# marbl/meryl

Hardware: AMD Instinct MI355X
Metric: distinct k-mers counted/sec (whole node) (higher is better)
Workload: dtype u64; 1 GPU; meryl count k=21 on synthetic short reads: 66666667 x 150 bp reads per GPU (10.00 Gbp per GPU, 30x of a 333333334 bp genome, 0.5% substitutions, 0.01% N), inputs resident in HBM; k=21, reads_per_gpu=66666667, bases_per_gpu=10066666717, n_distinct=1181289506, parallelism=1 GPU, transport=none (one GPU), n_instances=8648488363, w_prefix=18

## Files before the change

meryl_amd/build.py:

```python
import os
import shutil
import subprocess
import sys

HERE = os.path.dirname(os.path.abspath(__file__))
CSRC = os.path.join(HERE, "csrc")
LIB = os.path.join(HERE, "libmeryl_gpu_count.so")
SOURCES = ["mgc_kmer.hip", "mgc_sort.hip", "mgc_scan.hip", "mgc_finish.hip", "mgc_misc.hip", "mgc_parse.hip",
           "mgc_encode.hip", "mgc_decode.hip", "mgc_merge.hip", "mgc_merge_many.hip", "mgc_lookup.hip", "mgc_filter.hip", "mgc_import.hip", "mgc_analyze.hip", "mgc_value_hist.hip", "mgc_positions.hip",
           "mgc_api.cpp", "mgc_textfile.cpp", "mgc_import.cpp", "mgc_analyze.cpp", "mgc_dbfile.cpp", "mgc_positions.cpp", "mgc_count.cpp", "mgc_stream.cpp", "mgc_eval.cpp", "mgc_runs.cpp", "mgc_node.cpp", "meryl_db.cpp", "meryl_seq.cpp"]
HEADERS = ["mgc_device.h", "mgc_common.hpp", "mgc_compact.hpp", "mgc_bases.hpp", "mdb_layout.h", "mdb_statistics.hpp", "mgc_session.hpp", "mgc_devbuf.hpp", "mgc_dbfile.hpp", "mgc_hist_list.hpp", "mgc_clock.hpp", "mgc_chunk_ring.hpp", "mgc_bgzf.hpp", "mgc_runs.hpp", "mgc_lookup_dev.hpp", "mgc_import_dev.hpp", "mgc_analyze_dev.hpp", "mgc_positions_dev.hpp", "mgc_fastx.hpp", "mgc_label.hpp", "mgc_selector.hpp", "mgc_value.hpp", "mgc_route.hpp", "mgc_group_route.hpp",
           os.path.join("..", "..", "include", "meryl_gpu_count.h"),
           os.path.join("..", "..", "include", "meryl_db.h"), os.path.join("..", "..", "include", "meryl_seq.h"),
           os.path.join("..", "..", "include", "meryl_lookup.h"), os.path.join("..", "..", "include", "meryl_import.h"),
           os.path.join("..", "..", "include", "meryl_analyze.h"), os.path.join("..", "..", "include", "meryl_positions.h")]
OBJDIR = os.path.join(HERE, "build")
CFLAGS = ["--offload-arch=gfx950", "-O3", "-std=c++17", "-fPIC", "-pthread", "-Wall", "-Wno-unused-function"]
LFLAGS = ["--offload-arch=gfx950", "-shared", "-fPIC", "-pthread", "-no-hip-rt"]


def hipcc():
    for cand in (os.environ.get("HIPCC"), shutil.which("hipcc"), "/opt/rocm/bin/hipcc"):
        if cand and os.path.exists(cand):
            return cand
    raise RuntimeError("hipcc not found: the native library cannot be built")


def _sources():
    return [f for f in SOURCES if os.path.exists(os.path.join(CSRC, f))]


def _header_mtime():
    deps = [os.path.join(CSRC, f) for f in HEADERS if os.path.exists(os.path.join(CSRC, f))]
    deps.append(os.path.abspath(__file__))
    return max(os.path.getmtime(d) for d in deps)


def _obj(f):
    return os.path.join(OBJDIR, f + ".o")


def _stale_objects(force=False):
    ht = _header_mtime()
    out = []
    for f in _sources():
        o = _obj(f)
        if force or not os.path.exists(o) or os.path.getmtime(o) < max(os.path.getmtime(os.path.join(CSRC, f)), ht):
            out.append(f)
    return out


def _stale():
    if not os.path.exists(LIB):
        return True
    t = os.path.getmtime(LIB)
    if max([_header_mtime()] + [os.path.getmtime(os.path.join(CSRC, f)) for f in _sources()]) <= t:
        return False
    if _stale_objects():
        return True
    return any(os.path.getmtime(_obj(f)) > t for f in _sources())


CLI = os.path.join(HERE, "bin", "meryl")
LOOKUP_CLI = os.path.join(HERE, "bin", "meryl-lookup")
IMPORT_CLI = os.path.join(HERE, "bin", "meryl-import")
ANALYZE_CLI = os.path.join(HERE, "bin", "meryl-analyze")
POSITION_LOOKUP_CLI = os.path.join(HERE, "bin", "position-lookup")


def _build_front_end(source, out, force, verbose, headers=()):
    src = os.path.join(CSRC, source)
    newest = max(os.path.getmtime(os.path.join(CSRC, f)) for f in (source,) + tuple(headers))
    if (not force and os.path.exists(out) and os.path.getmtime(out) >= newest
            and os.path.getmtime(out) >= os.path.getmtime(LIB)):
        return out
    os.makedirs(os.path.dirname(out), exist_ok=True)
    rocm_lib = os.path.join(os.environ.get("ROCM_PATH", "/opt/rocm"), "lib")
    tmp = "%s.tmp%d" % (out, os.getpid())
    cmd = [hipcc(), "-O2", "-std=c++17", "-pthread", src, "-o", tmp, "-L" + HERE, "-lmeryl_gpu_count",
           "-Wl,-rpath,$ORIGIN/..", "-L" + rocm_lib, "-lamdhip64", "-Wl,-rpath," + rocm_lib, "-lz"]
    if verbose:
        print(" ".join(cmd), file=sys.stderr)
    subprocess.check_call(cmd)
    os.replace(tmp, out)
    return out


def build_cli(force=False, verbose=False):
    return _build_front_end("meryl_main.cpp", CLI, force, verbose)


def build_lookup_cli(force=False, verbose=False):
    return _build_front_end("meryl_lookup_main.cpp", LOOKUP_CLI, force, verbose, ("mgc_fastx.hpp",))


def build_import_cli(force=False, verbose=False):
    return _build_front_end("meryl_import_main.cpp", IMPORT_CLI, force, verbose)


def build_analyze_cli(force=False, verbose=False):
    return _build_front_end("meryl_analyze_main.cpp", ANALYZE_CLI, force, verbose)


def build_position_lookup_cli(force=False, verbose=False):
    return _build_front_end("position_lookup_main.cpp", POSITION_LOOKUP_CLI, force, verbose, ("mgc_fastx.hpp",))


def build(force=False, verbose=False):
    if not force and not _stale():
        build_cli(False, verbose)
        build_lookup_cli(False, verbose)
        build_import_cli(False, verbose)
        build_analyze_cli(False, verbose)
        build_position_lookup_cli(False, verbose)
        return LIB
    os.makedirs(OBJDIR, exist_ok=True)
    todo = _stale_objects(force)
    procs = []
    for f in todo:
        tmp = "%s.tmp%d" % (_obj(f), os.getpid())
        cmd = [hipcc()] + CFLAGS + ["-c", os.path.join(CSRC, f), "-o", tmp]
        if verbose:
            print(" ".join(cmd), file=sys.stderr)
        procs.append((f, tmp, cmd, subprocess.Popen(cmd)))
    failed = []
    for f, tmp, cmd, p in procs:
        if p.wait() != 0:
            failed.append(f)
        else:
            os.replace(tmp, _obj(f))
    if failed:
        raise subprocess.CalledProcessError(1, "hipcc -c " + " ".join(failed))
    tmp = "%s.tmp%d" % (LIB, os.getpid())
    cmd = [hipcc()] + LFLAGS + ["-o", tmp] + [_obj(f) for f in _sources()] + ["-lz"]
    if verbose:
        print(" ".join(cmd), file=sys.stderr)
    subprocess.check_call(cmd)
    os.replace(tmp, LIB)
    build_cli(True, verbose)
    build_lookup_cli(True, verbose)
    build_import_cli(True, verbose)
    build_analyze_cli(True, verbose)
    build_position_lookup_cli(True, verbose)
    return LIB


if __name__ == "__main__":
    print(build(force="--force" in sys.argv, verbose=True))
```

meryl_amd/csrc/mgc_finish.hip:

```cpp
#include "mgc_common.hpp"

#include <algorithm>
#include <type_traits>
#include <vector>

namespace mgc {


constexpr int RL_BLOCK = 256;
constexpr u64 RL_INF   = ~0ull;
template <typename K> struct RlTile { static constexpr int KPT = 16; };
template <> struct RlTile<K128>     { static constexpr int KPT = 8;  };

struct RleWs {
  u64 *total, *tile_offs, *tile_next, *scratch;
  u64  num_tiles;
};
static inline RleWs rle_ws(void *d_ws, uint64_t n, uint32_t key_words) {
  const uint64_t tile = (uint64_t)RL_BLOCK * (key_words == 2 ? RlTile<K128>::KPT : RlTile<u64>::KPT);
  RleWs w;
  w.num_tiles = (n + tile - 1) / tile;
  w.total     = reinterpret_cast<u64 *>(d_ws);
  w.tile_offs = w.total + 8;
  w.tile_next = w.tile_offs + w.num_tiles + 1;
  w.scratch   = w.tile_next + w.num_tiles + 1;
  return w;
}
size_t rle_workspace_bytes(uint64_t n) {
  const uint64_t t = (n + 2047) / 2048;
  return (size_t)(8 + 2 * (t + 1) + scan_scratch_elems(t + 1)) * sizeof(uint64_t);
}

template <typename K>
__global__ __launch_bounds__(RL_BLOCK)
void rle_count_kernel(const K *__restrict__ in, u64 n, u64 *__restrict__ tile_cnt, u64 *__restrict__ tile_first) {
  constexpr int KPT = RlTile<K>::KPT, TILE = RL_BLOCK * KPT;
  __shared__ u32 s_cnt[RL_BLOCK / 64];
  __shared__ u64 s_min[RL_BLOCK / 64];
  const u64 tile_base = (u64)blockIdx.x * TILE;
  u32 c = 0;
  u64 first = RL_INF;
#pragma unroll
  for (int j = 0; j < KPT; j++) {
    const u64 idx = tile_base + (u64)j * RL_BLOCK + threadIdx.x;
    if (idx < n) {
      const K key = in[idx];
      const bool head = (idx == 0) || KeyOps<K>::ne(in[idx - 1], key);
      if (head) { c++; if (idx < first) first = idx; }
    }
  }
#pragma unroll
  for (int d = 32; d >= 1; d >>= 1) {
    c += __shfl_down(c, d);
    const u64 o = __shfl_down(first, d);
    first = (o < first) ? o : first;
  }
  if (lane_id() == 0) { s_cnt[wave_id()] = c; s_min[wave_id()] = first; }
  __syncthreads();
  if (threadIdx.x == 0) {
    u32 tc = 0; u64 tf = RL_INF;
    for (int i = 0; i < RL_BLOCK / 64; i++) { tc += s_cnt[i]; tf = (s_min[i] < tf) ? s_min[i] : tf; }
    tile_cnt[blockIdx.x]   = tc;
    tile_first[blockIdx.x] = tf;
  }
}

__global__ void rle_set_tail_kernel(u64 *__restrict__ tile_offs, u64 *__restrict__ tile_next, u64 num_tiles, u64 n,
                                    const u64 *__restrict__ total) {
  tile_offs[num_tiles] = *total;
  tile_next[num_tiles] = n;
}

__device__ __forceinline__ u32 rl_pad(u32 i) { return i + (i >> 4); }

template <typename K>
__global__ __launch_bounds__(RL_BLOCK)
void rle_emit_kernel(const K *__restrict__ in, u64 n, const u64 *__restrict__ tile_offs,
                     const u64 *__restrict__ tile_next, const u64 *__restrict__ d_out_base, K *__restrict__ out_keys,
                     u32 *__restrict__ out_counts) {
  const u64 out_base0 = d_out_base ? *d_out_base : 0ull;
  constexpr int RL_KPT = RlTile<K>::KPT, RL_TILE = RL_BLOCK * RL_KPT;
  __shared__ K s_keys[RL_TILE + 1 + (RL_TILE + 1) / 16 + 1];
  __shared__ u32 s_tmp[RL_BLOCK / 64 + 1];
  __shared__ u64 s_wmin[RL_BLOCK / 64];
  const u32 tid = threadIdx.x, lane = lane_id(), w = wave_id();
  const u64 tile_base = (u64)blockIdx.x * RL_TILE;

  if (tid == 0) s_keys[rl_pad(0)] = (tile_base > 0) ? in[tile_base - 1] : KeyOps<K>::zero();
#pragma unroll
  for (int j = 0; j < RL_KPT; j++) {
    const u32 i   = (u32)j * RL_BLOCK + tid;
    const u64 idx = tile_base + i;
    s_keys[rl_pad(i + 1)] = (idx < n) ? in[idx] : KeyOps<K>::zero();
  }
  __syncthreads();

  K keys[RL_KPT];
  u32 flags = 0;
  K prev = s_keys[rl_pad(tid * RL_KPT)];
#pragma unroll
  for (int j = 0; j < RL_KPT; j++) {
    const u32 i   = tid * RL_KPT + j;
    const u64 idx = tile_base + i;
    keys[j] = s_keys[rl_pad(i + 1)];
    const bool head = (idx < n) && ((idx == 0) || KeyOps<K>::ne(keys[j], prev));
    flags |= (head ? 1u : 0u) << j;
    prev = keys[j];
  }

  const u32 c = __popc(flags);
  u32 tile_heads;
  const u32 slot0 = block_excl_scan<RL_BLOCK, u32>(c, s_tmp, &tile_heads);

  const u64 fh = flags ? (tile_base + (u64)tid * RL_KPT + (u32)(__ffs(flags) - 1)) : RL_INF;
  u64 x = fh;
#pragma unroll
  for (int d = 1; d < 64; d <<= 1) {
    const u64 y = __shfl_down(x, d);
    if ((int)lane + d < 64) x = (y < x) ? y : x;
  }
  if (lane == 0) s_wmin[w] = x;
  __syncthreads();
  u64 after = tile_next[blockIdx.x + 1];
  for (int ww = RL_BLOCK / 64 - 1; ww > (int)w; ww--) after = (s_wmin[ww] < after) ? s_wmin[ww] : after;
  u64 e = __shfl_down(x, 1);
  if (lane == 63) e = RL_INF;
  u64 next = (e < after) ? e : after;

  const u64 out_base = out_base0 + tile_offs[blockIdx.x] + slot0;
#pragma unroll
  for (int j = RL_KPT - 1; j >= 0; j--) {
    if ((flags >> j) & 1u) {
      const u64 idx  = tile_base + (u64)tid * RL_KPT + j;
      const u64 slot = out_base + __popc(flags & ((1u << j) - 1u));
      out_keys[slot]   = keys[j];
      out_counts[slot] = (u32)(next - idx);
      next = idx;
    }
  }
}

hipError_t launch_rle_count(const void *d_sorted, uint64_t n, uint32_t key_words, void *d_ws, hipStream_t st) {
  RleWs w = rle_ws(d_ws, n, key_words);
  if (n == 0) return hipMemsetAsync(w.total, 0, sizeof(u64), st);
  if (key_words == 2)
    hipLaunchKernelGGL(rle_count_kernel<K128>, dim3((uint32_t)w.num_tiles), dim3(RL_BLOCK), 0, st,
                       reinterpret_cast<const K128 *>(d_sorted), (u64)n, w.tile_offs, w.tile_next);
  else
    hipLaunchKernelGGL(rle_count_kernel<u64>, dim3((uint32_t)w.num_tiles), dim3(RL_BLOCK), 0, st,
                       reinterpret_cast<const u64 *>(d_sorted), (u64)n, w.tile_offs, w.tile_next);
  MGC_CHECK(hipGetLastError());
  MGC_CHECK(scan_u64_exclusive(w.tile_offs, w.num_tiles, w.scratch, w.total, st));
  MGC_CHECK(scan_u64_min_reverse(w.tile_next, w.num_tiles, w.scratch, (u64)n, st));
// ... 508 lines not shown
          won |= w ? (1u << j) : 0u;
          pending |= (act && !w && !dup) ? (1u << j) : 0u;
        }
      }
      while (pending) {
#pragma unroll
        for (int j = 0; j < KPT; j++) {
          if ((pending >> j) & 1u) {
            hh[j] = (hh[j] + 1) & smask;
            const u32 old = atomicCAS(&tk[hh[j]], EMPTY, (comp[j] << CNTB) | 1u);
            const bool w = old == EMPTY, dup = (old >> CNTB) == comp[j];
            if (dup) atomicAdd(&tk[hh[j]], 1u);
            if (w) won |= 1u << j;
            if (w || dup) pending &= ~(1u << j);
          }
        }
      }
      {
        u64 wm[KPT];
        u32 tot = 0;
#pragma unroll
        for (int j = 0; j < KPT; j++) { wm[j] = __ballot((won >> j) & 1u); tot += (u32)__popcll(wm[j]); }
        u32 base = 0;
        if (lane == 0) base = atomicAdd(&s_nd, tot);
        base = (u32)__builtin_amdgcn_readfirstlane((int)base);
#pragma unroll
        for (int j = 0; j < KPT; j++) {
          if (wm[j]) {
            if ((won >> j) & 1u)
              lst[base + __builtin_amdgcn_mbcnt_hi((u32)(wm[j] >> 32), __builtin_amdgcn_mbcnt_lo((u32)wm[j], 0u))] = (unsigned short)hh[j];
            base += (u32)__popcll(wm[j]);
          }
        }
      }
      }
      __syncthreads();
      HC_STAMP(1);
    }

    const u32 b1 = (R >= 2) ? bc[1] : 0u, b2 = (R >= 3) ? bc[2] : 0u, b3 = (R >= 4) ? bc[3] : 0u;
    const u64 a = a0;
    const u32 nslots = bn[R] <= (u32)CAP ? slots_for(bn[R]) : 256u;
    tag_keys(kcur, bn, comp);
    a0 = a0n;
#pragma unroll
    for (int j = 0; j <= R; j++) bc[j] = bn[j];
    unpack_bounds(bvec, a0n, bn);
    load_keys(a0n, bn[R], kcur);
    bvec = load_bvec(P + 3 * G);
    HC_STAMP(6);

    if (active) {
      const u32 D = s_nd;
      const bool big = D > (u32)BLOCK;
      u32 ent = 0, li = 0;
      if (!big) {
        if (tid < D) { ent = tk[lst[tid]]; li = atomicAdd(&s_bin[par][ent >> (CNTB + bshift)], 1u); }
      } else {
        for (u32 i = tid; i < D; i += BLOCK) {
          const u32 e = tk[lst[i]];
          srt[i] = e;
          lst[i] = (unsigned short)atomicAdd(&s_bin[par][e >> (CNTB + bshift)], 1u);
        }
      }
      __syncthreads();
      HC_STAMP(2);
      if (tid < 64) {
        uint4 c = reinterpret_cast<uint4 *>(s_bin[par])[tid];
        const u32 s4 = c.x + c.y + c.z + c.w;
        u32 x = s4;
#pragma unroll
        for (int d = 1; d < 64; d <<= 1) { const u32 y = __shfl_up(x, d); if ((int)lane >= d) x += y; }
        const u32 e0 = x - s4;
        reinterpret_cast<uint4 *>(s_bin[par])[tid] = make_uint4(e0, e0 + c.x, e0 + c.x + c.y, e0 + c.x + c.y + c.z);
        if (tid == 63) s_bin[par][BLOCK] = x;
      } else {
        uint4 *tk4 = reinterpret_cast<uint4 *>(tk);
        if (!big) for (u32 i = tid - 64; i < nslots / 4; i += BLOCK - 64) tk4[i] = make_uint4(EMPTY, EMPTY, EMPTY, EMPTY);
        for (u32 i = tid - 64; i < BLOCK; i += BLOCK - 64) s_bin[par ^ 1u][i] = 0;
        if (tid == 64) s_nd = 0;
      }
      cleared = nslots;
      __syncthreads();
      if (!big) {
        if (tid < D) srt[s_bin[par][ent >> (CNTB + bshift)] + li] = ent;
      } else {
        for (u32 i = tid; i < D; i += BLOCK) { const u32 e = srt[i]; tk[s_bin[par][e >> (CNTB + bshift)] + lst[i]] = e; }
      }
      __syncthreads();
      HC_STAMP(3);

      const u32 *sb = s_bin[par];
      const u32 *sorted = big ? tk : srt;
      u32 *kout = keys + a;
      u32 *cout = cnt_tmp + a;
      for (u32 p = tid; p < D; p += BLOCK) {
        const u32 e = sorted[p];
        const u32 b = e >> (CNTB + bshift), lo = sb[b], hi = sb[b + 1];
        u32 r = lo;
        for (u32 q = lo; q < hi; q++) r += (sorted[q] < e) ? 1u : 0u;
        const u32 tag = (R >= 2) ? (e >> (CNTB + low_bits)) : 0u;
        u32 dest = r;
        if (R >= 2) {
          const u32 sb_base = (tag == 0) ? 0u : ((tag == 1) ? b1 : ((tag == 2) ? b2 : b3));
          dest = sb_base + (r - sb[tag << (8u - TAGB)]);
        }
        kout[dest] = (e >> CNTB) & low_mask;
        cout[dest] = e & CNT_MASK;
      }
      if (tid < nsub) {
        const u32 dlo = sb[tid << (8u - TAGB)];
        const u32 dhi = (tid + 1 == (1u << TAGB)) ? D : sb[(tid + 1) << (8u - TAGB)];
        group_distinct[tr_index(g0 + tid, tr_a, tr_b)] = dhi - dlo;
      }
      if (big) {
        __syncthreads();
        uint4 *tk4 = reinterpret_cast<uint4 *>(tk);
        for (u32 i = tid; i < nslots / 4; i += BLOCK) tk4[i] = make_uint4(EMPTY, EMPTY, EMPTY, EMPTY);
        __syncthreads();
      }
      par ^= 1u;
      HC_STAMP(4);
    } else if (tid < nsub) {
      const u32 lo = (tid == 0) ? 0u : ((tid == 1) ? b1 : ((tid == 2) ? b2 : b3));
      const u32 hi = (tid + 1 == nsub) ? n : ((tid == 0) ? b1 : ((tid == 1) ? b2 : b3));
      u64 nj = hi - lo;
      if (n == 0xFFFFFFFFu) nj = starts[g0 + tid + 1] - starts[g0 + tid];
      if (nj == 0) group_distinct[tr_index(g0 + tid, tr_a, tr_b)] = 0;
      else if (nj <= max_size) retry_list[atomicAdd((unsigned long long *)retry_count, 1ull)] = (u32)(g0 + tid);
    }
    P += G;
    if (DBG) ph[7]++;
  }
  if (DBG && tid == 0 && blockIdx.x < 64)
    for (int i = 0; i < 8; i++) dbg[blockIdx.x * 8 + i] = ph[i];
#undef HC_STAMP
}

template <typename KT, int BLOCK, int KPC, int SLOTS, int DCAP, bool LIST, bool DBG, bool RETRY>
__global__ __launch_bounds__(BLOCK, (sizeof(KT) == 8 ? (SLOTS <= 2048 ? 5 : 1) : (SLOTS <= 2048 ? 8 : 2)))
void hash_count_stream_kernel(KT *__restrict__ keys, const u64 *__restrict__ starts, u64 ng, u64 max_size_, u32 low_bits,
                              u32 *__restrict__ cnt_tmp, u64 *__restrict__ group_distinct, u64 *__restrict__ dbg,
                              u32 tr_a, u32 tr_b, const u32 *__restrict__ visit, const u64 *__restrict__ visit_count,
                              u32 *__restrict__ retry_list, u64 *__restrict__ retry_count, u32 *__restrict__ error) {
  static_assert((SLOTS & (SLOTS - 1)) == 0 && SLOTS % (4 * BLOCK) == 0 && DCAP <= SLOTS && DCAP <= 65536 && BLOCK == 256, "table geometry");
  static_assert(sizeof(KT) == 4 || sizeof(KT) == 8, "32-bit words of a narrowed file, or whole 8-byte k-mers");
  constexpr bool W64 = sizeof(KT) == 8;
  constexpr u32 CNTB = 12u, CNT_MASK = (1u << CNTB) - 1u;
  constexpr KT EMPTY = (KT)~(KT)0;
  constexpr u32 CH = (u32)(BLOCK * KPC);
  constexpr u32 PROBE_MAX = 64u;
  __shared__ __attribute__((aligned(16))) KT tk[SLOTS];
  __shared__ __attribute__((aligned(16))) KT srt[DCAP];
  __shared__ unsigned short lst[DCAP];
  __shared__ __attribute__((aligned(16))) u32 s_bin[2][BLOCK + 4];
  __shared__ u32 s_nd, s_ovf;
  const u32 tid = threadIdx.x, lane = tid & 63u;
  const u32 G = gridDim.x;
  const KT  low_mask = (KT)((1ull << low_bits) - 1ull);
  const u32 bshift = low_bits - 8u;
  const u32 np = (u32)(LIST ? *visit_count : ng);
  const u32 max_size = (u32)max_size_;

  auto load_starts = [&](u32 P, u32 g) -> u32 {
    if (P >= np) return 0u;
    return (u32)starts[g + (lane ? 1u : 0u)];
  };
  auto unpack_bounds = [&](u32 bv, u32 &a, u32 &n) {
    a = (u32)__builtin_amdgcn_readlane((int)bv, 0);
    n = (u32)__builtin_amdgcn_readlane((int)bv, 1) - a;
  };
  auto load_gnum = [&](u32 P) -> u32 { return (LIST && P < np) ? visit[P] : 0u; };
  auto chunk_size = [&](u32 n) -> u32 {
    if (n == 0u || n > max_size) return 0u;
    u32 per = n;
    if (n > 2u * CH) per = ((n + 2u) * 43691u) >> 17;
    else if (n > CH) per = (n + 1u) >> 1;
    return (per + (u32)BLOCK - 1u) & ~((u32)BLOCK - 1u);
  };
  auto load_chunk = [&](u32 a, u32 cnt, KT (&kr)[KPC]) {
    const KT *src = keys + a;
#pragma unroll
    for (int j = 0; j < KPC; j++) {
      kr[j] = (KT)0;
      if ((u32)j * BLOCK < cnt) {
        const u32 last = cnt - 1u;
        const u32 idx = (u32)j * BLOCK + tid;
        kr[j] = src[idx < last ? idx : last];
      }
    }
  };
  auto slots_for = [&](u32 n) -> u32 {
    if (2u * n <= 256u) return 256u;
    const u32 s = 1u << (32 - __builtin_clz(2u * n - 1u));
    return s < (u32)SLOTS ? s : (u32)SLOTS;
  };

  u32 P = blockIdx.x;
  u32 a0, a1, g0, g1, n0, n1;
  KT  kcur[KPC], comp[KPC];
  KT  pre = (KT)0;
  g0 = LIST ? (u32)__builtin_amdgcn_readfirstlane((int)load_gnum(P)) : P;
  g1 = LIST ? (u32)__builtin_amdgcn_readfirstlane((int)load_gnum(P + G)) : P + G;
  u32 gb = LIST ? (u32)__builtin_amdgcn_readfirstlane((int)load_gnum(P + 2 * G)) : P + 2 * G;
  unpack_bounds(load_starts(P, g0), a0, n0);
  unpack_bounds(load_starts(P + G, g1), a1, n1);
  u32 csz = chunk_size(n0), off = 0;
  load_chunk(a0, csz < n0 ? csz : n0, kcur);
  u32 bvec = load_starts(P + 2 * G, gb);
  u32 gv = load_gnum(P + 3 * G);
  u32 par = 0;
  u32 cleared = (u32)SLOTS;
  constexpr u32 E16 = 16u / (u32)sizeof(KT);
  constexpr u32 ONES = 0xFFFFFFFFu;
  {
    uint4 *tk4 = reinterpret_cast<uint4 *>(tk);
    for (u32 i = tid; i < (u32)SLOTS / E16; i += BLOCK) tk4[i] = make_uint4(ONES, ONES, ONES, ONES);
    s_bin[0][tid] = 0; s_bin[1][tid] = 0;
    if (tid == 0) { s_nd = 0; s_ovf = 0; }
  }
  __syncthreads();

  u64 ph[8] = {0, 0, 0, 0, 0, 0, 0, 0}, t0 = 0;
#define HC_STAMP(i) do { if (DBG) { const u64 t = __builtin_readcyclecounter(); ph[i] += t - t0; t0 = t; } } while (0)
  while (P < np) {
    if (DBG) t0 = __builtin_readcyclecounter();
    const bool active = csz != 0u;
    const u32 rest = n0 - off;
    const u32 cnt = active ? (rest < csz ? rest : csz) : 0u;
    const bool last = !active || rest <= csz;
    const u32 slots = slots_for(n0);
    const u32 smask = slots - 1, sshift = 32 - (u32)__builtin_ctz(slots);
    const u32 probe_max = RETRY ? slots : PROBE_MAX;
    if constexpr (W64) { if (off == 0u) pre = kcur[0] & ~low_mask; }
#pragma unroll
    for (int j = 0; j < KPC; j++) {
      comp[j] = kcur[j] & low_mask;
      asm volatile("" : "+v"(comp[j]) :: "memory");
    }
    const u32 ncs = chunk_size(n1);
    u32 a2 = 0, n2 = 0, g2 = 0, g3 = 0;
    if (last) {
      unpack_bounds(bvec, a2, n2);
      g2 = gb;
      g3 = LIST ? (u32)__builtin_amdgcn_readfirstlane((int)gv) : P + 3 * G;
    }
    {
      const u32 la = last ? a1 : a0 + off + csz;
      const u32 lrest = last ? n1 : rest - csz, lcs = last ? ncs : csz;
      load_chunk(la, lrest < lcs ? lrest : lcs, kcur);
    }
    if (last) {
      bvec = load_starts(P + 3 * G, g3);
      gb = g3;
      if (LIST) gv = load_gnum(P + 4 * G);
    }
    HC_STAMP(6);
    if (active) {
      if (off == 0u && slots > cleared) {
        uint4 *tk4 = reinterpret_cast<uint4 *>(tk);
        for (u32 i = tid; i < (u32)SLOTS / E16; i += BLOCK) tk4[i] = make_uint4(ONES, ONES, ONES, ONES);
        __syncthreads();
      }
      HC_STAMP(0);
      u32 hh[KPC];
      u32 won = 0, pending = 0;
#pragma unroll
      for (int j = 0; j < KPC; j++) {
        if constexpr (W64) hh[j] = ((((u32)comp[j]) ^ ((u32)(comp[j] >> 32) * 0x85EBCA6Bu)) * 0x9E3779B1u) >> sshift;
        else               hh[j] = (comp[j] * 0x9E3779B1u) >> sshift;
        if ((u32)j * BLOCK < cnt) {
          const bool act = (u32)j * BLOCK + tid < cnt;
          KT old = (KT)0;
          if (act) old = atomicCAS(&tk[hh[j]], EMPTY, (KT)((comp[j] << CNTB) | (KT)1));
          const bool w = act && old == EMPTY, dup = act && !w && (old >> CNTB) == comp[j];
          if (dup) atomicAdd(reinterpret_cast<u32 *>(&tk[hh[j]]), 1u);
          won |= w ? (1u << j) : 0u;
          pending |= (act && !w && !dup) ? (1u << j) : 0u;
        }
      }
      u32 steps = 0;
      while (pending) {
#pragma unroll
        for (int j = 0; j < KPC; j++) {
          if ((pending >> j) & 1u) {
            hh[j] = (hh[j] + 1) & smask;
            const KT old = atomicCAS(&tk[hh[j]], EMPTY, (KT)((comp[j] << CNTB) | (KT)1));
            const bool w = old == EMPTY, dup = !w && (old >> CNTB) == comp[j];
            if (dup) atomicAdd(reinterpret_cast<u32 *>(&tk[hh[j]]), 1u);
            if (w) won |= 1u << j;
            if (w || dup) pending &= ~(1u << j);
          }
        }
        if (++steps > probe_max) { s_ovf = 1u; pending = 0; }
      }
      {
        u64 wm[KPC];
        u32 tot = 0;
#pragma unroll
        for (int j = 0; j < KPC; j++) { wm[j] = __ballot((won >> j) & 1u); tot += (u32)__popcll(wm[j]); }
        u32 base = 0;
        if (lane == 0) base = atomicAdd(&s_nd, tot);
        base = (u32)__builtin_amdgcn_readfirstlane((int)base);
        if (base + tot > (u32)DCAP) { if (lane == 0) s_ovf = 1u; }
        else {
#pragma unroll
          for (int j = 0; j < KPC; j++) {
            if (wm[j]) {
              if ((won >> j) & 1u)
                lst[base + __builtin_amdgcn_mbcnt_hi((u32)(wm[j] >> 32), __builtin_amdgcn_mbcnt_lo((u32)wm[j], 0u))] = (unsigned short)hh[j];
              base += (u32)__popcll(wm[j]);
            }
          }
        }
      }
      HC_STAMP(1);
    }
    if (!last) { off += csz; continue; }

    const u32 a = a0, g = g0, n = n0;
    const u32 nslots = slots_for(n1);
    if (active) __syncthreads();
    a0 = a1; n0 = n1; g0 = g1; off = 0; csz = ncs;
    a1 = a2; n1 = n2; g1 = g2;
    if (active) {
      const bool ovf = s_ovf != 0u;
      const u32 D = s_nd;
      if (!ovf) {
        const bool big = D > 2u * (u32)BLOCK;
        KT  ent0 = 0, ent1 = 0;
        u32 li0 = 0, li1 = 0;
        if (!big) {
          if (tid < D)              { ent0 = tk[lst[tid]];              li0 = atomicAdd(&s_bin[par][(u32)(ent0 >> (CNTB + bshift))], 1u); }
          if (tid + (u32)BLOCK < D) { ent1 = tk[lst[tid + (u32)BLOCK]]; li1 = atomicAdd(&s_bin[par][(u32)(ent1 >> (CNTB + bshift))], 1u); }
        } else {
          for (u32 i = tid; i < D; i += BLOCK) {
            const KT e = tk[lst[i]];
            srt[i] = e;
            lst[i] = (unsigned short)atomicAdd(&s_bin[par][(u32)(e >> (CNTB + bshift))], 1u);
          }
        }
        __syncthreads();
        HC_STAMP(2);
        if (tid < 64) {
          uint4 c = reinterpret_cast<uint4 *>(s_bin[par])[tid];
          const u32 s4 = c.x + c.y + c.z + c.w;
          u32 x = s4;
#pragma unroll
          for (int d = 1; d < 64; d <<= 1) { const u32 y = __shfl_up(x, d); if ((int)lane >= d) x += y; }
          const u32 e0 = x - s4;
          reinterpret_cast<uint4 *>(s_bin[par])[tid] = make_uint4(e0, e0 + c.x, e0 + c.x + c.y, e0 + c.x + c.y + c.z);
          if (tid == 63) s_bin[par][BLOCK] = x;
        } else {
          uint4 *tk4 = reinterpret_cast<uint4 *>(tk);
          if (!big) for (u32 i = tid - 64; i < nslots / E16; i += BLOCK - 64) tk4[i] = make_uint4(ONES, ONES, ONES, ONES);
          for (u32 i = tid - 64; i < BLOCK; i += BLOCK - 64) s_bin[par ^ 1u][i] = 0;
          if (tid == 64) s_nd = 0;
        }
        cleared = nslots;
        __syncthreads();
        if (!big) {
          if (tid < D)              srt[s_bin[par][(u32)(ent0 >> (CNTB + bshift))] + li0] = ent0;
          if (tid + (u32)BLOCK < D) srt[s_bin[par][(u32)(ent1 >> (CNTB + bshift))] + li1] = ent1;
        } else {
          for (u32 i = tid; i < D; i += BLOCK) { const KT e = srt[i]; tk[s_bin[par][(u32)(e >> (CNTB + bshift))] + lst[i]] = e; }
        }
        __syncthreads();
        HC_STAMP(3);

        const u32 *sb = s_bin[par];
        const KT *sorted = big ? tk : srt;
        KT *kout = keys + a;
        u32 *cout = cnt_tmp + a;
        for (u32 p = tid; p < D; p += BLOCK) {
          const KT  e = sorted[p];
          const u32 b = (u32)(e >> (CNTB + bshift)), lo = sb[b], hi = sb[b + 1];
          u32 r = lo;
          for (u32 q = lo; q < hi; q++) r += (sorted[q] < e) ? 1u : 0u;
          if constexpr (W64) kout[r] = pre | (e >> CNTB);
          else               kout[r] = e >> CNTB;
          cout[r] = (u32)e & CNT_MASK;
        }
        if (tid == 0) group_distinct[tr_index(g, tr_a, tr_b)] = D;
        if (big) {
          __syncthreads();
          uint4 *tk4 = reinterpret_cast<uint4 *>(tk);
          for (u32 i = tid; i < nslots / E16; i += BLOCK) tk4[i] = make_uint4(ONES, ONES, ONES, ONES);
          __syncthreads();
        }
        par ^= 1u;
        HC_STAMP(4);
      } else {
        __syncthreads();
        uint4 *tk4 = reinterpret_cast<uint4 *>(tk);
        for (u32 i = tid; i < (u32)SLOTS / E16; i += BLOCK) tk4[i] = make_uint4(ONES, ONES, ONES, ONES);
        if (tid == 0) {
          s_nd = 0; s_ovf = 0;
          if constexpr (RETRY) { atomicExch(error + 2, 1u); group_distinct[tr_index(g, tr_a, tr_b)] = 0; }
          else                 retry_list[atomicAdd((unsigned long long *)retry_count, 1ull)] = g;
        }
        cleared = (u32)SLOTS;
        __syncthreads();
      }
    } else if (n == 0u && tid == 0) {
      group_distinct[tr_index(g, tr_a, tr_b)] = 0;
    }
    P += G;
    if (DBG) ph[7]++;
  }
  if (DBG && tid == 0 && blockIdx.x < 64)
    for (int i = 0; i < 8; i++) dbg[blockIdx.x * 8 + i] = ph[i];
#undef HC_STAMP
}


template <typename KT, int BLOCK, int CAP, int SLOTS, bool WIDE, bool LIST>
__global__ __launch_bounds__(BLOCK, (sizeof(KT) >= 12 ? (CAP <= 768 ? 5 : 4) : (CAP <= 768 ? 6 : 5)))
void hash_countw_kernel(KT *__restrict__ keys, const u64 *__restrict__ starts, u64 ng, u64 max_size, u32 low_bits,
                        u32 *__restrict__ cnt_tmp, u64 *__restrict__ group_distinct,
                        const u32 *__restrict__ nz, const u64 *__restrict__ nz_count, u32 tr_a, u32 tr_b) {
  static_assert((SLOTS & (SLOTS - 1)) == 0 && SLOTS * 3 >= CAP * 4 && SLOTS % (4 * BLOCK) == 0 && CAP % BLOCK == 0 && CAP < 0xFFFF, "table geometry");
  static_assert(BLOCK == 256, "one bin per thread");
  constexpr bool K16 = sizeof(KT) >= 12;
  constexpr bool IS96 = sizeof(KT) == 12;
  static_assert(K16 || !WIDE, "WIDE is a property of 16- and 12-byte keys");
  constexpr int KPT = CAP / BLOCK;
  constexpr u32 EMPTY = 0x0000FFFFu;
  __shared__ __attribute__((aligned(16))) u64 dlo[CAP];
  __shared__ __attribute__((aligned(16))) u64 dhi[WIDE ? CAP : 2];
  __shared__ __attribute__((aligned(16))) u32 tw[SLOTS];
  __shared__ __attribute__((aligned(16))) u32 srt[CAP];
  constexpr bool DB = !(WIDE && CAP > 768);
  __shared__ __attribute__((aligned(16))) u32 s_bin[DB ? 2 : 1][BLOCK + 4];
  __shared__ u32 s_nd;
  unsigned short *lst = reinterpret_cast<unsigned short *>(srt);
  const u32 tid = threadIdx.x, lane = tid & 63u;
  const u64 G = gridDim.x;
  const u64 mask_lo = (low_bits >= 64) ? ~0ull : ((1ull << low_bits) - 1ull);
  const u64 mask_hi = (low_bits <= 64) ? 0ull : ((low_bits >= 128) ? ~0ull : ((1ull << (low_bits - 64)) - 1ull));
  const u32 bshift = low_bits > 8 ? low_bits - 8 : 0;
  const u64 np = LIST ? *nz_count : ng;

  auto bin_of = [&](u64 lo, u64 hi) -> u32 {
    if (WIDE) return bshift >= 64 ? (u32)(hi >> (bshift - 64)) : (u32)((hi << (64 - bshift)) | (lo >> bshift));
    return (u32)(lo >> bshift);
  };
  auto rdlane64 = [&](u64 v, int l) -> u64 {
    const u32 lo = (u32)__builtin_amdgcn_readlane((int)(u32)v, l), hi = (u32)__builtin_amdgcn_readlane((int)(u32)(v >> 32), l);
    return ((u64)hi << 32) | lo;
  };
  auto load_g = [&](u64 Q) -> u32 {
    if (Q >= np) return 0xFFFFFFFFu;
    return LIST ? nz[Q] : (u32)Q;
  };
  auto load_bvec = [&](u32 g) -> u64 {
    if (g == 0xFFFFFFFFu) return 0ull;
    return starts[(u64)g + (lane ? 1u : 0u)];
  };
  auto unpack_bounds = [&](u64 bv, u64 &a0, u32 &n) {
    a0 = rdlane64(bv, 0);
    const u64 d = rdlane64(bv, 1) - a0;
    n = d > 0xFFFFFFFFull ? 0xFFFFFFFFu : (u32)d;
  };
  auto load_keys = [&](u64 a0, u32 n, KT (&kr)[KPT]) {
    const bool fits = (u64)n <= max_size;
#pragma unroll
    for (int j = 0; j < KPT; j++) {
      if constexpr (IS96) { kr[j].w[0] = 0u; kr[j].w[1] = 0u; kr[j].w[2] = 0u; } else if constexpr (K16) { kr[j].lo = 0ull; kr[j].hi = 0ull; } else kr[j] = 0ull;
      if (fits && (u32)j * BLOCK < n) {
        const KT *src = keys + a0 + (u32)j * BLOCK;
        const u32 last = n - 1u - (u32)j * BLOCK;
        kr[j] = src[tid < last ? tid : last];
      }
    }
  };
  auto slots_for = [&](u32 n) -> u32 {
    u32 s = 256;
    while (s < n + n / 4 && s < (u32)SLOTS) s <<= 1;
    return s;
  };
  u64 klo[KPT], khi[K16 ? KPT : 1], pre_lo = 0, pre_hi = 0;
  KT kcur[KPT];
  auto consume = [&]() {
    if constexpr (IS96) { pre_lo = KeyOps<K96>::low64(kcur[0]) & ~mask_lo; pre_hi = (u64)kcur[0].w[2] & ~mask_hi; }
    else if constexpr (K16) { pre_lo = kcur[0].lo & ~mask_lo; pre_hi = kcur[0].hi & ~mask_hi; }
    else pre_lo = kcur[0] & ~mask_lo;
#pragma unroll
    for (int j = 0; j < KPT; j++) {
      if constexpr (IS96) {
        klo[j] = KeyOps<K96>::low64(kcur[j]) & mask_lo; khi[j] = (u64)kcur[j].w[2] & mask_hi;
        asm volatile("" : "+v"(klo[j]) :: "memory"); asm volatile("" : "+v"(khi[j]) :: "memory");
      } else if constexpr (K16) {
        klo[j] = kcur[j].lo & mask_lo; khi[j] = kcur[j].hi & mask_hi;
        asm volatile("" : "+v"(klo[j]) :: "memory"); asm volatile("" : "+v"(khi[j]) :: "memory");
      } else { klo[j] = kcur[j] & mask_lo; asm volatile("" : "+v"(klo[j]) :: "memory"); }
    }
  };

  u64 P = blockIdx.x;
  u32 g0 = (u32)__builtin_amdgcn_readfirstlane((int)load_g(P)), g1 = (u32)__builtin_amdgcn_readfirstlane((int)load_g(P + G)),
      g2 = (u32)__builtin_amdgcn_readfirstlane((int)load_g(P + 2 * G));
  u64 a0, a0n;
  u32 nc, nn;
  unpack_bounds(load_bvec(g0), a0, nc);
  load_keys(a0, nc, kcur);
  u64 bvec = load_bvec(g1);
  consume();
  unpack_bounds(bvec, a0n, nn);
  load_keys(a0n, nn, kcur);
  bvec = load_bvec(g2);
  u32 gv = load_g(P + 3 * G);
  u32 par = 0;
  u32 cleared = (u32)SLOTS;
  {
    uint4 *tw4 = reinterpret_cast<uint4 *>(tw);
    for (u32 i = tid; i < (u32)SLOTS / 4; i += BLOCK) tw4[i] = make_uint4(EMPTY, EMPTY, EMPTY, EMPTY);
    s_bin[0][tid] = 0; if constexpr (DB) s_bin[1][tid] = 0;
    if (tid == 0) s_nd = 0;
  }
  __syncthreads();

  while (P < np) {
    const u32 n = nc;
    const bool active = n != 0 && (u64)n <= max_size;
    const u32 slots = slots_for(n);
    if (active) {
      u32 hh[KPT];
      const u32 smask = slots - 1, sshift = 32 - (u32)__builtin_ctz(slots);
      if (slots > cleared) {
        uint4 *tw4 = reinterpret_cast<uint4 *>(tw);
        for (u32 i = tid; i < (u32)SLOTS / 4; i += BLOCK) tw4[i] = make_uint4(EMPTY, EMPTY, EMPTY, EMPTY);
      }
#pragma unroll
      for (int j = 0; j < KPT; j++) {
        const u64 mix = K16 ? (klo[j] ^ (khi[K16 ? j : 0] * 0xD6E8FEB86659FD93ull)) * 0x9E3779B97F4A7C15ull : klo[j] * 0x9E3779B97F4A7C15ull;
        hh[j] = (u32)(mix >> 32) >> sshift;
        if ((u32)j * BLOCK + tid < n) { dlo[(u32)j * BLOCK + tid] = klo[j]; if (WIDE) dhi[(u32)j * BLOCK + tid] = khi[K16 ? j : 0]; }
      }
      if constexpr (!DB) s_bin[0][tid] = 0;
      __syncthreads();
      auto same = [&](u32 rep, int j) -> bool { return dlo[rep] == klo[j] && (!WIDE || dhi[rep] == khi[K16 ? j : 0]); };
      u32 won = 0, pending = 0;
#pragma unroll
      for (int j = 0; j < KPT; j++) {
        if ((u32)j * BLOCK < n) {
          const bool act = (u32)j * BLOCK + tid < n;
          u32 old = 0;
          if (act) old = atomicCAS(&tw[hh[j]], EMPTY, (1u << 16) | ((u32)j * BLOCK + tid));
          const bool w = act && old == EMPTY;
          const bool dup = act && !w && same(old & 0xFFFFu, j);
          if (dup) atomicAdd(&tw[hh[j]], 1u << 16);
          won |= w ? (1u << j) : 0u;
          pending |= (act && !w && !dup) ? (1u << j) : 0u;
        }
// ... 1466 lines not shown
```

Before: 11.88 billion distinct k-mers/s.

## Queue hash-probe collisions per wave and compact table by bucket scan

Reworks the streaming hash-count kernel. A collided insert is no longer retried in a per-thread loop; it is pushed into a small per-wave shared-memory queue and drained cooperatively, which cuts divergent probe loops. Distinct keys are counted into the radix bins at insert time, so the separate won-list (lst) and the big/small compaction paths are dropped. The table is then scanned vectorised and cleared in the same pass to scatter entries into sorted order. The costs are extra shared memory for the queues, a full-table scan even for sparse groups, and more atomics on the bins during insertion.

```diff
diff --git a/meryl_amd/build.py b/meryl_amd/build.py
--- a/meryl_amd/build.py
+++ b/meryl_amd/build.py
@@ -9,7 +9,7 @@
 SOURCES = ["mgc_kmer.hip", "mgc_sort.hip", "mgc_scan.hip", "mgc_finish.hip", "mgc_misc.hip", "mgc_parse.hip",
            "mgc_encode.hip", "mgc_decode.hip", "mgc_merge.hip", "mgc_merge_many.hip", "mgc_lookup.hip", "mgc_filter.hip", "mgc_import.hip", "mgc_analyze.hip", "mgc_value_hist.hip", "mgc_positions.hip",
            "mgc_api.cpp", "mgc_textfile.cpp", "mgc_import.cpp", "mgc_analyze.cpp", "mgc_dbfile.cpp", "mgc_positions.cpp", "mgc_count.cpp", "mgc_stream.cpp", "mgc_eval.cpp", "mgc_runs.cpp", "mgc_node.cpp", "meryl_db.cpp", "meryl_seq.cpp"]
-HEADERS = ["mgc_device.h", "mgc_common.hpp", "mgc_compact.hpp", "mgc_bases.hpp", "mdb_layout.h", "mdb_statistics.hpp", "mgc_session.hpp", "mgc_devbuf.hpp", "mgc_dbfile.hpp", "mgc_hist_list.hpp", "mgc_clock.hpp", "mgc_chunk_ring.hpp", "mgc_bgzf.hpp", "mgc_runs.hpp", "mgc_lookup_dev.hpp", "mgc_import_dev.hpp", "mgc_analyze_dev.hpp", "mgc_positions_dev.hpp", "mgc_fastx.hpp", "mgc_label.hpp", "mgc_selector.hpp", "mgc_value.hpp", "mgc_route.hpp", "mgc_group_route.hpp",
+HEADERS = ["mgc_device.h", "mgc_common.hpp", "mgc_compact.hpp", "mgc_bases.hpp", "mgc_stream_geom.hpp", "mdb_layout.h", "mdb_statistics.hpp", "mgc_session.hpp", "mgc_devbuf.hpp", "mgc_dbfile.hpp", "mgc_hist_list.hpp", "mgc_clock.hpp", "mgc_chunk_ring.hpp", "mgc_bgzf.hpp", "mgc_runs.hpp", "mgc_lookup_dev.hpp", "mgc_import_dev.hpp", "mgc_analyze_dev.hpp", "mgc_positions_dev.hpp", "mgc_fastx.hpp", "mgc_label.hpp", "mgc_selector.hpp", "mgc_value.hpp", "mgc_route.hpp", "mgc_group_route.hpp",
            os.path.join("..", "..", "include", "meryl_gpu_count.h"),
            os.path.join("..", "..", "include", "meryl_db.h"), os.path.join("..", "..", "include", "meryl_seq.h"),
            os.path.join("..", "..", "include", "meryl_lookup.h"), os.path.join("..", "..", "include", "meryl_import.h"),
diff --git a/meryl_amd/csrc/mgc_finish.hip b/meryl_amd/csrc/mgc_finish.hip
--- a/meryl_amd/csrc/mgc_finish.hip
+++ b/meryl_amd/csrc/mgc_finish.hip
@@ -1,4 +1,5 @@
 #include "mgc_common.hpp"
+#include "mgc_stream_geom.hpp"
 
 #include <algorithm>
 #include <type_traits>
@@ -813,10 +814,11 @@
   constexpr u32 PROBE_MAX = 64u;
   __shared__ __attribute__((aligned(16))) KT tk[SLOTS];
   __shared__ __attribute__((aligned(16))) KT srt[DCAP];
-  __shared__ unsigned short lst[DCAP];
   __shared__ __attribute__((aligned(16))) u32 s_bin[2][BLOCK + 4];
-  __shared__ u32 s_nd, s_ovf;
+  __shared__ KT s_q[(BLOCK / 64) * (int)STREAM_QCAP];
+  __shared__ u32 s_ovf;
   const u32 tid = threadIdx.x, lane = tid & 63u;
+  const u32 wave = (u32)__builtin_amdgcn_readfirstlane((int)(tid >> 6));
   const u32 G = gridDim.x;
   const KT  low_mask = (KT)((1ull << low_bits) - 1ull);
   const u32 bshift = low_bits - 8u;
@@ -832,13 +834,7 @@
     n = (u32)__builtin_amdgcn_readlane((int)bv, 1) - a;
   };
   auto load_gnum = [&](u32 P) -> u32 { return (LIST && P < np) ? visit[P] : 0u; };
-  auto chunk_size = [&](u32 n) -> u32 {
-    if (n == 0u || n > max_size) return 0u;
-    u32 per = n;
-    if (n > 2u * CH) per = ((n + 2u) * 43691u) >> 17;
-    else if (n > CH) per = (n + 1u) >> 1;
-    return (per + (u32)BLOCK - 1u) & ~((u32)BLOCK - 1u);
-  };
+  auto chunk_size = [&](u32 n) -> u32 { return stream_chunk_size(n, max_size, CH, (u32)BLOCK); };
   auto load_chunk = [&](u32 a, u32 cnt, KT (&kr)[KPC]) {
     const KT *src = keys + a;
 #pragma unroll
@@ -851,12 +847,6 @@
       }
     }
   };
-  auto slots_for = [&](u32 n) -> u32 {
-    if (2u * n <= 256u) return 256u;
-    const u32 s = 1u << (32 - __builtin_clz(2u * n - 1u));
-    return s < (u32)SLOTS ? s : (u32)SLOTS;
-  };
-
   u32 P = blockIdx.x;
   u32 a0, a1, g0, g1, n0, n1;
   KT  kcur[KPC], comp[KPC];
@@ -867,22 +857,55 @@
   unpack_bounds(load_starts(P, g0), a0, n0);
   unpack_bounds(load_starts(P + G, g1), a1, n1);
   u32 csz = chunk_size(n0), off = 0;
+  u32 ncs = chunk_size(n1);
+  u32 slots = csz ? stream_slots_for(n0, (u32)SLOTS) : 256u, smask = slots - 1u, sshift = 32u - (u32)__builtin_ctz(slots), probe_max = RETRY ? slots : PROBE_MAX;
   load_chunk(a0, csz < n0 ? csz : n0, kcur);
   u32 bvec = load_starts(P + 2 * G, gb);
   u32 gv = load_gnum(P + 3 * G);
   u32 par = 0;
-  u32 cleared = (u32)SLOTS;
   constexpr u32 E16 = 16u / (u32)sizeof(KT);
   constexpr u32 ONES = 0xFFFFFFFFu;
+  auto vec_entry = [](const uint4 &q, int i) -> KT {
+    if constexpr (W64) return i == 0 ? (((KT)q.y << 32) | (KT)q.x) : (((KT)q.w << 32) | (KT)q.z);
+    else               return i == 0 ? q.x : (i == 1 ? q.y : (i == 2 ? q.z : q.w));
+  };
+  auto home_of = [](KT c, u32 sshift) -> u32 {
+    if constexpr (W64) return ((((u32)c) ^ ((u32)(c >> 32) * 0x85EBCA6Bu)) * 0x9E3779B1u) >> sshift;
+    else               return (c * 0x9E3779B1u) >> sshift;
+  };
+  auto drain_queue = [&](u32 &qn, u32 smask, u32 sshift, u32 probe_max) {
+    __builtin_amdgcn_fence(__ATOMIC_RELEASE, "wavefront");
+    __builtin_amdgcn_wave_barrier();
+    for (u32 b = 0; b < qn; b += 64u) {
+      if (b + lane < qn) {
+        const KT c = s_q[stream_queue_index(wave, b, lane)];
+        u32 h = home_of(c, sshift), steps = 0;
+        bool pend = true;
+        do {
+          h = (h + 1) & smask;
+          const KT old = atomicCAS(&tk[h], EMPTY, (KT)((c << CNTB) | (KT)1));
+          const bool w = old == EMPTY, dup = !w && (old >> CNTB) == c;
+          if (dup) atomicAdd(reinterpret_cast<u32 *>(&tk[h]), 1u);
+          if (w)   atomicAdd(&s_bin[par][(u32)(c >> bshift)], 1u);
+          if (w || dup) pend = false;
+          if (++steps > probe_max) { s_ovf = 1u; pend = false; }
+        } while (pend);
+      }
+    }
+    __builtin_amdgcn_wave_barrier();
+    __builtin_amdgcn_fence(__ATOMIC_ACQUIRE, "wavefront");
+    qn = 0;
+  };
   {
     uint4 *tk4 = reinterpret_cast<uint4 *>(tk);
     for (u32 i = tid; i < (u32)SLOTS / E16; i += BLOCK) tk4[i] = make_uint4(ONES, ONES, ONES, ONES);
     s_bin[0][tid] = 0; s_bin[1][tid] = 0;
-    if (tid == 0) { s_nd = 0; s_ovf = 0; }
+    if (tid == 0) s_ovf = 0;
   }
   __syncthreads();
 
   u64 ph[8] = {0, 0, 0, 0, 0, 0, 0, 0}, t0 = 0;
+  u32 qn = 0;
 #define HC_STAMP(i) do { if (DBG) { const u64 t = __builtin_readcyclecounter(); ph[i] += t - t0; t0 = t; } } while (0)
   while (P < np) {
     if (DBG) t0 = __builtin_readcyclecounter();
@@ -890,16 +913,12 @@
     const u32 rest = n0 - off;
     const u32 cnt = active ? (rest < csz ? rest : csz) : 0u;
     const bool last = !active || rest <= csz;
-    const u32 slots = slots_for(n0);
-    const u32 smask = slots - 1, sshift = 32 - (u32)__builtin_ctz(slots);
-    const u32 probe_max = RETRY ? slots : PROBE_MAX;
     if constexpr (W64) { if (off == 0u) pre = kcur[0] & ~low_mask; }
 #pragma unroll
     for (int j = 0; j < KPC; j++) {
       comp[j] = kcur[j] & low_mask;
       asm volatile("" : "+v"(comp[j]) :: "memory");
     }
-    const u32 ncs = chunk_size(n1);
     u32 a2 = 0, n2 = 0, g2 = 0, g3 = 0;
     if (last) {
       unpack_bounds(bvec, a2, n2);
@@ -918,119 +937,107 @@
     }
     HC_STAMP(6);
     if (active) {
-      if (off == 0u && slots > cleared) {
-        uint4 *tk4 = reinterpret_cast<uint4 *>(tk);
-        for (u32 i = tid; i < (u32)SLOTS / E16; i += BLOCK) tk4[i] = make_uint4(ONES, ONES, ONES, ONES);
-        __syncthreads();
-      }
       HC_STAMP(0);
-      u32 hh[KPC];
-      u32 won = 0, pending = 0;
-#pragma unroll
-      for (int j = 0; j < KPC; j++) {
-        if constexpr (W64) hh[j] = ((((u32)comp[j]) ^ ((u32)(comp[j] >> 32) * 0x85EBCA6Bu)) * 0x9E3779B1u) >> sshift;
-        else               hh[j] = (comp[j] * 0x9E3779B1u) >> sshift;
-        if ((u32)j * BLOCK < cnt) {
-          const bool act = (u32)j * BLOCK + tid < cnt;
-          KT old = (KT)0;
-          if (act) old = atomicCAS(&tk[hh[j]], EMPTY, (KT)((comp[j] << CNTB) | (KT)1));
-          const bool w = act && old == EMPTY, dup = act && !w && (old >> CNTB) == comp[j];
-          if (dup) atomicAdd(reinterpret_cast<u32 *>(&tk[hh[j]]), 1u);
-          won |= w ? (1u << j) : 0u;
-          pending |= (act && !w && !dup) ? (1u << j) : 0u;
-        }
-      }
-      u32 steps = 0;
-      while (pending) {
-#pragma unroll
-        for (int j = 0; j < KPC; j++) {
-          if ((pending >> j) & 1u) {
-            hh[j] = (hh[j] + 1) & smask;
-            const KT old = atomicCAS(&tk[hh[j]], EMPTY, (KT)((comp[j] << CNTB) | (KT)1));
-            const bool w = old == EMPTY, dup = !w && (old >> CNTB) == comp[j];
-            if (dup) atomicAdd(reinterpret_cast<u32 *>(&tk[hh[j]]), 1u);
-            if (w) won |= 1u << j;
-            if (w || dup) pending &= ~(1u << j);
-          }
-        }
-        if (++steps > probe_max) { s_ovf = 1u; pending = 0; }
-      }
-      {
-        u64 wm[KPC];
-        u32 tot = 0;
-#pragma unroll
-        for (int j = 0; j < KPC; j++) { wm[j] = __ballot((won >> j) & 1u); tot += (u32)__popcll(wm[j]); }
-        u32 base = 0;
-        if (lane == 0) base = atomicAdd(&s_nd, tot);
-        base = (u32)__builtin_amdgcn_readfirstlane((int)base);
-        if (base + tot > (u32)DCAP) { if (lane == 0) s_ovf = 1u; }
-        else {
-#pragma unroll
-          for (int j = 0; j < KPC; j++) {
-            if (wm[j]) {
-              if ((won >> j) & 1u)
-                lst[base + __builtin_amdgcn_mbcnt_hi((u32)(wm[j] >> 32), __builtin_amdgcn_mbcnt_lo((u32)wm[j], 0u))] = (unsigned short)hh[j];
-              base += (u32)__popcll(wm[j]);
-            }
-          }
-        }
-      }
+      auto first_probe = [&](auto PARTIAL, const KT c, const bool act) {
+        const u32 h = home_of(c, sshift);
+        KT old = (KT)0;
+        bool pend;
+        if constexpr (decltype(PARTIAL)::value) {
+          if (act) old = atomicCAS(&tk[h], EMPTY, (KT)((c << CNTB) | (KT)1));
+          const bool w = act && old == EMPTY, dup = act && !w && (old >> CNTB) == c;
+          if (dup) atomicAdd(reinterpret_cast<u32 *>(&tk[h]), 1u);
+          if (w)   atomicAdd(&s_bin[par][(u32)(c >> bshift)], 1u);
+          pend = act && !w && !dup;
+        } else {
+          old = atomicCAS(&tk[h], EMPTY, (KT)((c << CNTB) | (KT)1));
+          const bool w = old == EMPTY, dup = !w && (old >> CNTB) == c;
+          if (dup) atomicAdd(reinterpret_cast<u32 *>(&tk[h]), 1u);
+          if (w)   atomicAdd(&s_bin[par][(u32)(c >> bshift)], 1u);
+          pend = !w && !dup;
+        }
+        const u64 pm = __ballot(pend);
+        if (pm) {
+          const u32 pc = (u32)__popcll(pm);
+          if (stream_queue_must_drain(qn, pc)) drain_queue(qn, smask, sshift, probe_max);
+          if (pend) s_q[stream_queue_index(wave, qn, __builtin_amdgcn_mbcnt_hi((u32)(pm >> 32), __builtin_amdgcn_mbcnt_lo((u32)pm, 0u)))] = c;
+          qn += pc;
+        }
+      };
+      const u32 full_rows = cnt / (u32)BLOCK;
+#pragma unroll
+      for (int j = 0; j < KPC; j++)
+        if ((u32)j < full_rows) first_probe(std::false_type(), comp[j], true);
+      if (cnt & ((u32)BLOCK - 1u)) {
+        KT c = comp[0];
+#pragma unroll
+        for (int j = 1; j < KPC; j++) c = (full_rows == (u32)j) ? comp[j] : c;
+        first_probe(std::true_type(), c, full_rows * (u32)BLOCK + tid < cnt);
+      }
+      if (last && qn) drain_queue(qn, smask, sshift, probe_max);
       HC_STAMP(1);
     }
     if (!last) { off += csz; continue; }
 
     const u32 a = a0, g = g0, n = n0;
-    const u32 nslots = slots_for(n1);
+    const u32 nvec = slots / E16;
     if (active) __syncthreads();
     a0 = a1; n0 = n1; g0 = g1; off = 0; csz = ncs;
-    a1 = a2; n1 = n2; g1 = g2;
+    a1 = a2; n1 = n2; g1 = g2; ncs = chunk_size(n2);
+    slots = csz ? stream_slots_for(n0, (u32)SLOTS) : 256u;
+    smask = slots - 1u; sshift = 32u - (u32)__builtin_ctz(slots); probe_max = RETRY ? slots : PROBE_MAX;
     if (active) {
-      const bool ovf = s_ovf != 0u;
-      const u32 D = s_nd;
+      uint4 *tk4 = reinterpret_cast<uint4 *>(tk);
+      bool ovf = s_ovf != 0u;
+      u32 D = 0;
       if (!ovf) {
-        const bool big = D > 2u * (u32)BLOCK;
-        KT  ent0 = 0, ent1 = 0;
-        u32 li0 = 0, li1 = 0;
-        if (!big) {
-          if (tid < D)              { ent0 = tk[lst[tid]];              li0 = atomicAdd(&s_bin[par][(u32)(ent0 >> (CNTB + bshift))], 1u); }
-          if (tid + (u32)BLOCK < D) { ent1 = tk[lst[tid + (u32)BLOCK]]; li1 = atomicAdd(&s_bin[par][(u32)(ent1 >> (CNTB + bshift))], 1u); }
-        } else {
-          for (u32 i = tid; i < D; i += BLOCK) {
-            const KT e = tk[lst[i]];
-            srt[i] = e;
-            lst[i] = (unsigned short)atomicAdd(&s_bin[par][(u32)(e >> (CNTB + bshift))], 1u);
-          }
-        }
-        __syncthreads();
         HC_STAMP(2);
         if (tid < 64) {
-          uint4 c = reinterpret_cast<uint4 *>(s_bin[par])[tid];
+          const uint4 c = reinterpret_cast<uint4 *>(s_bin[par])[tid];
           const u32 s4 = c.x + c.y + c.z + c.w;
           u32 x = s4;
 #pragma unroll
           for (int d = 1; d < 64; d <<= 1) { const u32 y = __shfl_up(x, d); if ((int)lane >= d) x += y; }
           const u32 e0 = x - s4;
-          reinterpret_cast<uint4 *>(s_bin[par])[tid] = make_uint4(e0, e0 + c.x, e0 + c.x + c.y, e0 + c.x + c.y + c.z);
-          if (tid == 63) s_bin[par][BLOCK] = x;
+          u32 *S = s_bin[par] + 1u + 4u * tid;
+          S[0] = e0; S[1] = e0 + c.x; S[2] = e0 + c.x + c.y; S[3] = e0 + c.x + c.y + c.z;
+          if (tid == 0)  s_bin[par][0] = 0;
+          if (tid == 63) s_bin[par][BLOCK + 1] = x;
         } else {
-          uint4 *tk4 = reinterpret_cast<uint4 *>(tk);
-          if (!big) for (u32 i = tid - 64; i < nslots / E16; i += BLOCK - 64) tk4[i] = make_uint4(ONES, ONES, ONES, ONES);
           for (u32 i = tid - 64; i < BLOCK; i += BLOCK - 64) s_bin[par ^ 1u][i] = 0;
-          if (tid == 64) s_nd = 0;
-        }
-        cleared = nslots;
+        }
         __syncthreads();
-        if (!big) {
-          if (tid < D)              srt[s_bin[par][(u32)(ent0 >> (CNTB + bshift))] + li0] = ent0;
-          if (tid + (u32)BLOCK < D) srt[s_bin[par][(u32)(ent1 >> (CNTB + bshift))] + li1] = ent1;
-        } else {
-          for (u32 i = tid; i < D; i += BLOCK) { const KT e = srt[i]; tk[s_bin[par][(u32)(e >> (CNTB + bshift))] + lst[i]] = e; }
+        D = s_bin[par][BLOCK + 1];
+        ovf = D > (u32)DCAP;
+      }
+      if (!ovf) {
+        const uint4 ones4 = make_uint4(ONES, ONES, ONES, ONES);
+        for (u32 v = tid; v < nvec; v += 2u * BLOCK) {
+          const bool two = v + (u32)BLOCK < nvec;
+          const uint4 q0 = tk4[v];
+          uint4 q1 = ones4;
+          if (two) q1 = tk4[v + (u32)BLOCK];
+          tk4[v] = ones4;
+          if (two) tk4[v + (u32)BLOCK] = ones4;
+          u32 pos0[E16], pos1[E16];
+#pragma unroll
+          for (int i = 0; i < (int)E16; i++) {
+            const KT e0 = vec_entry(q0, i), e1 = vec_entry(q1, i);
+            pos0[i] = 0; pos1[i] = 0;
+            if (e0 != EMPTY) pos0[i] = atomicAdd(&s_bin[par][1u + (u32)(e0 >> (CNTB + bshift))], 1u);
+            if (e1 != EMPTY) pos1[i] = atomicAdd(&s_bin[par][1u + (u32)(e1 >> (CNTB + bshift))], 1u);
+          }
+#pragma unroll
+          for (int i = 0; i < (int)E16; i++) {
+            const KT e0 = vec_entry(q0, i), e1 = vec_entry(q1, i);
+            if (e0 != EMPTY) srt[pos0[i]] = e0;
+            if (e1 != EMPTY) srt[pos1[i]] = e1;
+          }
         }
         __syncthreads();
         HC_STAMP(3);
 
         const u32 *sb = s_bin[par];
-        const KT *sorted = big ? tk : srt;
+        const KT *sorted = srt;
         KT *kout = keys + a;
         u32 *cout = cnt_tmp + a;
         for (u32 p = tid; p < D; p += BLOCK) {
@@ -1043,24 +1050,17 @@
           cout[r] = (u32)e & CNT_MASK;
         }
         if (tid == 0) group_distinct[tr_index(g, tr_a, tr_b)] = D;
-        if (big) {
-          __syncthreads();
-          uint4 *tk4 = reinterpret_cast<uint4 *>(tk);
-          for (u32 i = tid; i < nslots / E16; i += BLOCK) tk4[i] = make_uint4(ONES, ONES, ONES, ONES);
-          __syncthreads();
-        }
         par ^= 1u;
         HC_STAMP(4);
       } else {
         __syncthreads();
-        uint4 *tk4 = reinterpret_cast<uint4 *>(tk);
         for (u32 i = tid; i < (u32)SLOTS / E16; i += BLOCK) tk4[i] = make_uint4(ONES, ONES, ONES, ONES);
+        s_bin[0][tid] = 0; s_bin[1][tid] = 0;
         if (tid == 0) {
-          s_nd = 0; s_ovf = 0;
+          s_ovf = 0;
           if constexpr (RETRY) { atomicExch(error + 2, 1u); group_distinct[tr_index(g, tr_a, tr_b)] = 0; }
           else                 retry_list[atomicAdd((unsigned long long *)retry_count, 1ull)] = g;
         }
-        cleared = (u32)SLOTS;
         __syncthreads();
       }
     } else if (n == 0u && tid == 0) {
diff --git a/meryl_amd/csrc/mgc_stream_geom.hpp b/meryl_amd/csrc/mgc_stream_geom.hpp
--- /dev/null
+++ b/meryl_amd/csrc/mgc_stream_geom.hpp
@@ -0,0 +1,30 @@
+#pragma once
+#include <cstdint>
+
+#if defined(__HIPCC__) || defined(__CUDACC__)
+#define MGC_GEOM_FN __host__ __device__ __forceinline__
+#else
+#define MGC_GEOM_FN inline
+#endif
+
+namespace mgc {
+
+MGC_GEOM_FN uint32_t stream_chunk_size(uint32_t n, uint32_t max_size, uint32_t ch, uint32_t block) {
+  if (n == 0u || n > max_size) return 0u;
+  uint32_t per = n;
+  if (n > 2u * ch) per = ((n + 2u) * 43691u) >> 17;
+  else if (n > ch) per = (n + 1u) >> 1;
+  return (per + block - 1u) & ~(block - 1u);
+}
+
+MGC_GEOM_FN uint32_t stream_slots_for(uint32_t n, uint32_t table) {
+  if (2u * n <= 256u) return 256u;
+  const uint32_t s = 1u << (32 - __builtin_clz(2u * n - 1u));
+  return s < table ? s : table;
+}
+
+constexpr uint32_t STREAM_QCAP = 128u;
+MGC_GEOM_FN bool     stream_queue_must_drain(uint32_t fill, uint32_t row_keys) { return fill + row_keys > STREAM_QCAP; }
+MGC_GEOM_FN uint32_t stream_queue_index(uint32_t wave, uint32_t fill, uint32_t rank_in_row) { return wave * STREAM_QCAP + fill + rank_in_row; }
+
+}
```

New measurement: 12.06 billion distinct k-mers/s (median of 6 runs). +1.5%, better.
